# WPCLab/OpenSeg3D

Hardware: AMD Instinct MI355X
Metric: points/sec fwd+bwd, Waymo 1-sweep ~180k pts @0.1m voxel; logit parity (higher is better)
Workload: dtype f32 storage/accumulate, bf16x3 products; 1 GPU; waymo_one_sweep (BASELINE configs[1]): synthetic scene, 174633 pts/step/GPU, voxel [0.1, 0.1, 0.1], grid [1440, 1440, 64], fwd (attention dropout p=0.1, DropPath) + criterion (ohem_ce+lovasz on 3 heads) + bwd + SGD step; mode=fwdbwd, segmentor=segformer, voxels=108690, parallelism=dp1

## Files before the change

__graft_entry__.py:

```python
import os
import subprocess
import sys

ROOT = os.path.dirname(os.path.abspath(__file__))
CSRC = os.path.join(ROOT, "openseg3d_amd", "csrc")
LIB = os.path.join(CSRC, "libseg3d_hip.so")
HIP_SOURCES = ["scan.hip", "voxelize.hip", "group.hip", "rulebook.hip", "spconv.hip", "spconv_split.hip", "linear_stream.hip", "linear_x6.hip", "spconv_dma.hip", "spconv_tile.hip", "wgrad_split.hip", "wgrad_dense.hip", "wgrad_dense_lds.hip", "window.hip",
               "attention.hip", "attention_fused.hip", "attention_fused_bwd.hip", "attention_small.hip", "rownorm.hip", "segment.hip", "knn.hip", "knn_attention.hip", "class_context.hip", "loss.hip", "lovasz.hip"]
HIPCC_FLAGS = ["--offload-arch=gfx950", "-O3", "-std=c++17", "-fPIC", "-ffp-contract=off",
               "-fhip-fp32-correctly-rounded-divide-sqrt", "-Wall", "-Wno-unused-function"]


def _stale(target, deps):
    if not os.path.exists(target):
        return True
    t = os.path.getmtime(target)
    return any(os.path.getmtime(d) > t for d in deps)


def build_hip(force=False, verbose=False):
    hipcc = os.environ.get("HIPCC", "/opt/rocm/bin/hipcc")
    common = [os.path.join(CSRC, "common.hpp"), os.path.join(CSRC, "attn_common.hpp"), os.path.join(CSRC, "attn_dropout.hpp"), os.path.join(CSRC, "attn_fused.hpp"),
              os.path.join(ROOT, "include", "seg3d_hip.h")]
    objs = []
    procs = []
    for src in HIP_SOURCES:
        s = os.path.join(CSRC, src)
        o = os.path.join(CSRC, src.replace(".hip", ".o"))
        objs.append(o)
        if force or _stale(o, [s] + common):
            cmd = [hipcc] + HIPCC_FLAGS + ["-c", s, "-o", o]
            if verbose:
                print(" ".join(cmd))
            procs.append((src, subprocess.Popen(cmd, stdout=subprocess.PIPE, stderr=subprocess.STDOUT)))
    failed = False
    for src, p in procs:
        out, _ = p.communicate()
        if p.returncode != 0:
            failed = True
            sys.stderr.write(f"--- hipcc failed on {src}\n{out.decode()}\n")
        elif verbose and out.strip():
            print(out.decode())
    if failed:
        raise RuntimeError("hipcc failed")
    if force or procs or _stale(LIB, objs):
        subprocess.check_call([hipcc, "--offload-arch=gfx950", "-shared", "-fPIC", "-o", LIB] + objs)
    return LIB


def build():
    build_hip()
    subprocess.check_call(["make", "-C", os.path.join(ROOT, "oracle")], stdout=subprocess.DEVNULL)
    sys.path.insert(0, ROOT)
    import openseg3d_amd
    from openseg3d_amd import _lib
# ... 12 lines not shown
```

include/seg3d_hip.h:

```cpp
#ifndef SEG3D_HIP_H
#define SEG3D_HIP_H

#include <stddef.h>
#include <stdint.h>

#ifdef __cplusplus
extern "C" {
#endif

#define SEG3D_OK 0
#define SEG3D_EINVAL (-1)
#define SEG3D_EWORKSPACE (-2)
#define SEG3D_ELAUNCH (-3)

#define SEG3D_REDUCE_SUM 0
#define SEG3D_REDUCE_MEAN 1
#define SEG3D_REDUCE_MAX 2

int seg3d_abi_version(void);

const char* seg3d_last_error(void);

int seg3d_grid_size(const float* voxel_size, const float* range, int32_t* grid_xyz);

// ... 105 lines not shown
int seg3d_linear_pack_weight_f32(const float* weight, int32_t cin, int32_t cout, int32_t transpose,
                                 void* w_packed, void* stream);
int seg3d_linear_fwd_f32(const float* x, int64_t m, const void* w_packed, const float* bias ,
                         int32_t cin, int32_t cout, float* y, void* stream);
size_t seg3d_linear_packed_bytes_x6(int32_t cin, int32_t cout);
int seg3d_linear_pack_weight_x6(const float* weight, int32_t cin, int32_t cout, int32_t transpose, void* w_packed,
                                void* stream);
int seg3d_linear_fwd_x6(const float* x, int64_t m, const void* w_packed, const float* bias ,
                        const float* scale , const float* shift , int32_t relu, int32_t cin,
                        int32_t cout, float* y, void* stream);

typedef struct {
  const float* src;
  void* dst;
  int32_t cin, cout;
  int32_t kk, transpose, flip, reserved;
  int64_t first_block;
} seg3d_pack_job;
int seg3d_pack_weights_batched(const void* jobs, int32_t n_jobs, int64_t total_blocks, void* stream);

size_t seg3d_linear_packed_bytes(int32_t cin, int32_t cout, int32_t transpose);
int seg3d_linear_pack_weight(const float* weight, int32_t cin, int32_t cout, int32_t transpose,
                             void* w_packed, void* stream);
int seg3d_linear_fwd(const float* x, int64_t m, const void* w_packed, const float* bias ,
                     const float* addend , int32_t cin, int32_t cout,
                     float* y, void* stream);
int seg3d_linear_fwd_sum(const float* x, const float* x_add, int64_t m, const void* w_packed, const float* bias,
                         int32_t cin, int32_t cout, float* y, void* stream);
int seg3d_linear_layernorm_fwd(const float* x, int64_t m, const void* w_packed, const float* bias, const float* res,
                               const float* gamma, const float* beta, float eps, int32_t cin, int32_t cout, float* y,
                               void* stream);
int seg3d_linear_fwd_mul(const float* x, int64_t m, const void* w_packed, const float* factor, int32_t cin, int32_t cout,
                         float* y, void* stream);

size_t seg3d_window_partition_workspace_bytes(int64_t m, int32_t batch_size, const int32_t* nwin_xyz);
int seg3d_window_partition(const int32_t* coords, int64_t m, int32_t batch_size,
                           const int32_t* win_xyz, const int32_t* nwin_xyz, const int32_t* shift_xyz,
                           int32_t n_levels, const int32_t* level_lo, const int32_t* level_hi,
                           const int32_t* level_cap, int32_t* win_id, int32_t* in_win, int32_t* rank,
                           int32_t* level, int32_t* slot, int32_t* tok, int32_t* win_start,
                           int32_t* win_count, int32_t* win_tile0, int32_t* tile_item,
                           int32_t* qg_item, int32_t* counts, void* workspace,
                           size_t workspace_bytes, void* stream);

int seg3d_pos_embed(const int32_t* in_win, int64_t m, const int32_t* win_xyz ,
                    const float* inv_freq, int32_t c, float* pos, void* stream);

int seg3d_window_attn_supported(int32_t heads, int32_t dh);
size_t seg3d_window_attn_workspace_bytes(int64_t m, int32_t n_tiles, int32_t heads, int32_t dh);
int seg3d_window_attn_fwd(const float* q, const float* k, const float* v, int32_t ldq, int32_t ldk,
                          int32_t ldv, const int32_t* tok, const int32_t* win_start,
                          const int32_t* win_count, const int32_t* win_tile0,
                          const int32_t* tile_item, int32_t n_tiles, const int32_t* qg_item,
                          int32_t n_qgroups, int64_t m, int32_t n_windows, int32_t heads, int32_t dh,
                          const float* tau, float tau_min, float dropout_p, uint64_t dropout_seed, float* out,
                          float* lse, void* workspace, size_t workspace_bytes, void* stream);
int seg3d_window_attn_bwd(const float* q, const float* k, const float* v, int32_t ldq, int32_t ldk,
                          int32_t ldv, const float* out, const float* dout, const float* lse,
                          const int32_t* tok, const int32_t* win_start, const int32_t* win_count,
                          const int32_t* win_tile0, const int32_t* tile_item, int32_t n_tiles,
                          const int32_t* qg_item, int32_t n_qgroups, int64_t m, int32_t n_windows,
                          int32_t heads, int32_t dh, const float* tau,
                          float tau_min, float dropout_p, uint64_t dropout_seed, float* dq, float* dk,
                          float* dv, int32_t lddq, int32_t lddk,
                          int32_t lddv, float* dtau, void* workspace, size_t workspace_bytes,
                          void* stream);
// ... 105 lines not shown
```

openseg3d_amd/_lib.py:

```python
import ctypes
import os
import re

_HERE = os.path.dirname(os.path.abspath(__file__))
LIB_PATH = os.path.join(_HERE, "csrc", "libseg3d_hip.so")
HEADER_PATH = os.path.join(os.path.dirname(_HERE), "include", "seg3d_hip.h")

OK, EINVAL, EWORKSPACE, ELAUNCH = 0, -1, -2, -3
REDUCE_SUM, REDUCE_MEAN, REDUCE_MAX = 0, 1, 2
ABI_VERSION = 40

_p, _i32, _i64, _sz, _f = ctypes.c_void_p, ctypes.c_int32, ctypes.c_int64, ctypes.c_size_t, ctypes.c_float
_u64 = ctypes.c_uint64

SIGNATURES = {
    "seg3d_abi_version": (ctypes.c_int, []),
    "seg3d_last_error": (ctypes.c_char_p, []),
    "seg3d_grid_size": (ctypes.c_int, [_p, _p, _p]),
    "seg3d_voxelize_workspace_bytes": (_sz, [_i64]),
    "seg3d_voxelize_f32": (ctypes.c_int, [_p, _i64, _i32, _i32, _i32, _p, _p, _p, _p, _p, _p, _sz, _p]),
    "seg3d_voxelize_f64": (ctypes.c_int, [_p, _i64, _i32, _i32, _i32, _p, _p, _p, _p, _p, _p, _sz, _p]),
    "seg3d_voxelize_host_workspace_bytes": (_sz, [_i64]),
    "seg3d_voxelize_host_f32": (ctypes.c_int, [_p, _i64, _i32, _i32, _i32, _p, _p, _p, _p, _p, _p, _sz]),
    "seg3d_voxelize_host_f64": (ctypes.c_int, [_p, _i64, _i32, _i32, _i32, _p, _p, _p, _p, _p, _p, _sz]),
    "seg3d_cart2polar_f32": (ctypes.c_int, [_p, _i64, _i32, _i32, _p, _p]),
    "seg3d_cart2polar_f64": (ctypes.c_int, [_p, _i64, _i32, _i32, _p, _p]),
    "seg3d_group_index_workspace_bytes": (_sz, [_i64, _i64]),
    "seg3d_group_index": (ctypes.c_int, [_p, _i64, _i64, _p, _p, _p, _p, _sz, _p]),
    "seg3d_coord_hash_bytes": (_sz, [_i64]),
    "seg3d_coord_hash_build": (ctypes.c_int, [_p, _i64, _p, _p, _sz, _p]),
    "seg3d_rulebook_subm": (ctypes.c_int, [_p, _i64, _p, _p, _sz, _p, _p]),
    "seg3d_downsample_workspace_bytes": (_sz, [_i32, _p]),
    "seg3d_downsample_coords": (ctypes.c_int, [_p, _i64, _p, _i32, _p, _p, _i64, _p, _p, _sz, _p]),
    "seg3d_rulebook_strided": (ctypes.c_int, [_p, _i64, _i64, _p, _p, _sz, _p, _p, _p]),
    "seg3d_spconv_packed_bytes": (_sz, [_i32, _i32, _i32]),
    "seg3d_spconv_pack_weight": (ctypes.c_int, [_p, _i32, _i32, _i32, _p, _p]),
    "seg3d_spconv_fwd": (ctypes.c_int, [_p, _p, _i64, _i64, _p, _i32, _p, _i32, _i32, _p, _p, _p]),
    "seg3d_spconv_fwd_act": (ctypes.c_int, [_p, _p, _i64, _i64, _p, _i32, _p, _p, _i32, _i32, _i32, _p, _p, _p]),
    "seg3d_spconv_fwd_act_bf16": (ctypes.c_int, [_p, _i32, _p, _i64, _i64, _p, _i32, _p, _p, _i32, _i32, _i32, _p, _p, _p]),
    "seg3d_spconv_presplit_bytes": (_sz, [_i64, _i32]),
    "seg3d_spconv_presplit": (ctypes.c_int, [_p, _i64, _i32, _p, _p]),
    "seg3d_spconv_fwd_presplit": (ctypes.c_int, [_p, _p, _i64, _i64, _p, _i32, _p, _p, _i32, _i32, _i32, _p, _p, _p]),
    "seg3d_conv_plan_bytes": (_sz, [_i64]),
    "seg3d_conv_plan_workspace_bytes": (_sz, [_i64]),
    "seg3d_conv_plan_build": (ctypes.c_int, [_p, _p, _i64, _p, _p, _sz, _p]),
    "seg3d_spconv_tiled_supported": (_i32, [_i32, _i32]),
    "seg3d_spconv_fwd_tiled": (ctypes.c_int, [_p, _p, _p, _i64, _i64, _p, _i32, _p, _p, _i32, _i32, _i32, _p, _p]),
    "seg3d_spconv_fwd_tiled_bf16": (ctypes.c_int, [_p, _i32, _p, _p, _i64, _i64, _p, _i32, _p, _p, _i32, _i32, _i32, _p, _p]),
    "seg3d_debug_set_conv_nbt": (ctypes.c_int, [_i32]),
    "seg3d_debug_set_linear_stream": (ctypes.c_int, [_i32]),
    "seg3d_spconv_wgrad_workspace_bytes": (_sz, [_i64, _i32, _i32]),
    "seg3d_spconv_wgrad": (ctypes.c_int, [_p, _p, _p, _i64, _i64, _i32, _i32, _i32, _p, _p, _sz, _p]),
    "seg3d_spconv_wgrad_partials": (ctypes.c_int, [_p, _p, _p, _i64, _i64, _i32, _i32, _p, _sz, _p, _p]),
    "seg3d_spconv_wgrad_partials_xbf16": (ctypes.c_int, [_p, _p, _p, _i64, _i64, _i32, _i32, _p, _sz, _p, _p]),
    "seg3d_linear_wgrad_partials_xbf16": (ctypes.c_int, [_p, _p, _i64, _i32, _i32, _i32, _p, ctypes.c_size_t, _p, _p]),
    "seg3d_linear_packed_bytes_f32": (ctypes.c_size_t, [_i32, _i32]),
    "seg3d_linear_pack_weight_f32": (ctypes.c_int, [_p, _i32, _i32, _i32, _p, _p]),
    "seg3d_linear_fwd_f32": (ctypes.c_int, [_p, _i64, _p, _p, _i32, _i32, _p, _p]),
    "seg3d_debug_set_wgrad_lds": (ctypes.c_int, [_i32]),
    "seg3d_linear_packed_bytes_x6": (ctypes.c_size_t, [_i32, _i32]),
    "seg3d_linear_pack_weight_x6": (ctypes.c_int, [_p, _i32, _i32, _i32, _p, _p]),
    "seg3d_linear_fwd_x6": (ctypes.c_int, [_p, _i64, _p, _p, _p, _p, _i32, _i32, _i32, _p, _p]),
    "seg3d_pack_weights_batched": (ctypes.c_int, [_p, _i32, _i64, _p]),
    "seg3d_linear_wgrad_workspace_bytes": (ctypes.c_size_t, [_i64, _i32, _i32]),
    "seg3d_linear_wgrad": (ctypes.c_int, [_p, _p, _i64, _i32, _i32, _p, _p, _p, ctypes.c_size_t, _p]),
    "seg3d_linear_wgrad_partials": (ctypes.c_int, [_p, _p, _i64, _i32, _i32, _i32, _p, ctypes.c_size_t, _p, _p]),
    "seg3d_reduce_partials": (ctypes.c_int, [_p, _i32, _i64, _i64, _p, _p, _p]),
    "seg3d_reduce_partials_batched": (ctypes.c_int, [_p, _i32, _i64, _p]),
    "seg3d_linear_packed_bytes": (_sz, [_i32, _i32, _i32]),
    "seg3d_linear_pack_weight": (ctypes.c_int, [_p, _i32, _i32, _i32, _p, _p]),
    "seg3d_linear_fwd": (ctypes.c_int, [_p, _i64, _p, _p, _p, _i32, _i32, _p, _p]),
    "seg3d_linear_fwd_sum": (ctypes.c_int, [_p, _p, _i64, _p, _p, _i32, _i32, _p, _p]),
    "seg3d_linear_fwd_mul": (ctypes.c_int, [_p, _i64, _p, _p, _i32, _i32, _p, _p]),
    "seg3d_linear_layernorm_fwd": (ctypes.c_int, [_p, _i64, _p, _p, _p, _p, _p, ctypes.c_float, _i32, _i32, _p, _p]),
    "seg3d_window_partition_workspace_bytes": (_sz, [_i64, _i32, _p]),
    "seg3d_window_partition": (ctypes.c_int, [_p, _i64, _i32, _p, _p, _p, _i32, _p, _p, _p,
                                              _p, _p, _p, _p, _p, _p, _p, _p, _p, _p, _p, _p, _p, _sz, _p]),
    "seg3d_pos_embed": (ctypes.c_int, [_p, _i64, _p, _p, _i32, _p, _p]),
    "seg3d_window_attn_supported": (ctypes.c_int, [_i32, _i32]),
    "seg3d_window_attn_workspace_bytes": (_sz, [_i64, _i32, _i32, _i32]),
    "seg3d_window_attn_fwd": (ctypes.c_int, [_p, _p, _p, _i32, _i32, _i32, _p, _p, _p, _p, _p, _i32, _p, _i32,
                                             _i64, _i32, _i32, _i32, _p, _f, _f, _u64, _p, _p, _p, _sz, _p]),
    "seg3d_window_attn_bwd": (ctypes.c_int, [_p, _p, _p, _i32, _i32, _i32, _p, _p, _p, _p, _p, _p, _p, _p, _i32, _p,
                                             _i32, _i64, _i32, _i32, _i32, _p, _f, _f, _u64, _p, _p, _p, _i32, _i32, _i32,
                                             _p, _p, _sz, _p]),
    "seg3d_layernorm_fwd": (ctypes.c_int, [_p, _p, _p, _p, _p, _f, _i64, _i32, _p, _p, _p, _p]),
    "seg3d_layernorm_bwd_workspace_bytes": (ctypes.c_size_t, [_i64, _i32]),
    "seg3d_layernorm_bwd": (ctypes.c_int, [_p, _p, _p, _p, _p, _p, _i64, _i32, _p, _p, _p, _p, ctypes.c_size_t, _p]),
    "seg3d_layernorm_bwd_partials": (ctypes.c_int, [_p, _p, _p, _p, _p, _p, _i64, _i32, _p, _p, ctypes.c_size_t, _p, _p]),
    "seg3d_batchnorm_workspace_bytes": (ctypes.c_size_t, [_i64, _i32]),
    "seg3d_colstats": (ctypes.c_int, [_p, _i64, _i32, _p, _p, ctypes.c_size_t, _p]),
    "seg3d_batchnorm_stats": (ctypes.c_int, [_p, _i64, _i32, _f, _p, _p, _f, _p, _p, _p, _p, ctypes.c_size_t, _p]),
    "seg3d_affine_act": (ctypes.c_int, [_p, _p, _p, _p, _i32, _i64, _i32, _p, _p]),
    "seg3d_gelu_fwd": (ctypes.c_int, [_p, _i64, _p, _p, _p]),
    "seg3d_batchnorm_bwd": (ctypes.c_int, [_p, _p, _p, _p, _p, _p, _i32, _i64, _i32, _p, _p, _p, _p, ctypes.c_size_t, _p]),
    "seg3d_batchnorm_bwd_reduce": (ctypes.c_int, [_p, _p, _p, _p, _p, _i32, _i64, _i32, _p, _p, ctypes.c_size_t, _p]),
    "seg3d_batchnorm_bwd_apply": (ctypes.c_int, [_p, _p, _p, _p, _p, _p, _p, _p, _i32, _i64, _i32, _p, _p, _p]),
    "seg3d_segment_reduce_fwd": (ctypes.c_int, [_p, _i32, _p, _p, _i64, _i32, _p, _p, _p]),
    "seg3d_segment_reduce_bwd": (ctypes.c_int, [_p, _i32, _p, _i64, _p, _p, _i64, _i32, _p, _p]),
    "seg3d_voxel_majority_labels": (ctypes.c_int, [_p, _p, _p, _i64, _i32, _p, _p]),
    "seg3d_cross_entropy_workspace_bytes": (ctypes.c_size_t, [_i64]),
    "seg3d_cross_entropy_fwd": (ctypes.c_int, [_p, _p, _i64, _i32, _i64, _f, _p, _p, _p, ctypes.c_size_t, _p]),
    "seg3d_cross_entropy_bwd": (ctypes.c_int, [_p, _p, _p, _p, _p, _i64, _i32, _p, _p]),
    "seg3d_lovasz_workspace_bytes": (ctypes.c_size_t, [_i64, _i32]),
    "seg3d_lovasz_softmax_fwd": (ctypes.c_int, [_p, _p, _i64, _i32, _i64, _i32, _p, _p, _p, _p, _p, ctypes.c_size_t, _p]),
    "seg3d_lovasz_softmax_bwd": (ctypes.c_int, [_p, _p, _p, _p, _i64, _i32, _p, _p]),
# ... 64 lines not shown
```

openseg3d_amd/csrc/rownorm.hip:

```cpp
#include "common.hpp"

namespace {

constexpr int kThreads = 256;
constexpr int kMaxBlocks = 2048;
constexpr int kLnBwdMaxBlocks = 1024;

struct RowMap {
    int quads;
    int p;
    int items;
};

inline RowMap row_map(int c) {
    RowMap m;
    m.quads = c / 4;
    m.items = (m.quads + 63) / 64;
    int need = (m.quads + m.items - 1) / m.items;
    m.p = 8;
    while (m.p < need) m.p <<= 1;
    return m;
}

__device__ __forceinline__ float group_sum(float v, int p) {
    for (int off = 1; off < p; off <<= 1) v += __shfl_xor(v, off, SEG3D_WAVE);
    return v;
}

template <int ITEMS>
__global__ __launch_bounds__(kThreads) void ln_fwd_kernel(const float* __restrict__ x, const float* __restrict__ res,
                                                          const float* __restrict__ gamma, const float* __restrict__ beta,
                                                          const float* __restrict__ rowscale, float eps, int64_t m, int c,
                                                          RowMap rm, float* __restrict__ y, float* __restrict__ mean,
// ... 208 lines not shown
        for (; b + 96 < nblocks; b += 128) {
            s0 += part[(int64_t)b * c2 + i];
            s1 += part[(int64_t)(b + 32) * c2 + i];
            s2 += part[(int64_t)(b + 64) * c2 + i];
            s3 += part[(int64_t)(b + 96) * c2 + i];
        }
        for (; b < nblocks; b += 32) s0 += part[(int64_t)b * c2 + i];
        s = (s0 + s1) + (s2 + s3);
    }
    red[q][col] = s;
    __syncthreads();
    float t = red[0][col];
#pragma unroll
    for (int k = 1; k < 32; ++k) t += red[k][col];
    __syncthreads();
    return t;
}

__global__ __launch_bounds__(1024) void col_sums_finish(const float* __restrict__ part, int nblocks, int c,
                                                        float* __restrict__ sums ) {
    __shared__ float red[32][33];
    const int i = blockIdx.x * 32 + (threadIdx.x & 31);
    const float t = col_partial_sum(part, nblocks, 2 * c, i, red);
    if ((threadIdx.x >> 5) == 0 && i < 2 * c) sums[i] = t;
}

__global__ __launch_bounds__(kThreads) void gelu_fwd_kernel(const float* __restrict__ h, int64_t quads, float* __restrict__ g,
                                                            float* __restrict__ gp) {
    for (int64_t t = (int64_t)blockIdx.x * kThreads + threadIdx.x; t < quads; t += (int64_t)gridDim.x * kThreads) {
        const float4 v = reinterpret_cast<const float4*>(h)[t];
        const float in[4] = {v.x, v.y, v.z, v.w};
        float o[4], d[4];
#pragma unroll
        for (int i = 0; i < 4; ++i) {
            const float cdf = 0.5f * (1.0f + erff(in[i] * 0.70710678118654752440f));
            o[i] = in[i] * cdf;
            d[i] = cdf + in[i] * (0.39894228040143267794f * __expf(-0.5f * in[i] * in[i]));
        }
        reinterpret_cast<float4*>(g)[t] = make_float4(o[0], o[1], o[2], o[3]);
        if (gp) reinterpret_cast<float4*>(gp)[t] = make_float4(d[0], d[1], d[2], d[3]);
    }
}

__global__ __launch_bounds__(kThreads) void affine_act_kernel(const float* __restrict__ x, const float* __restrict__ res,
                                                              const float* __restrict__ scale, const float* __restrict__ shift,
                                                              int relu, int64_t total_quads, int quads, float* __restrict__ y) {
    for (int64_t t = (int64_t)blockIdx.x * kThreads + threadIdx.x; t < total_quads; t += (int64_t)gridDim.x * kThreads) {
        const int q = (int)(t % quads);
        const float4 xv = reinterpret_cast<const float4*>(x)[t];
        const float4 s = *reinterpret_cast<const float4*>(scale + 4 * q);
        const float4 b = *reinterpret_cast<const float4*>(shift + 4 * q);
        float4 o = make_float4(xv.x * s.x + b.x, xv.y * s.y + b.y, xv.z * s.z + b.z, xv.w * s.w + b.w);
        if (res) {
            const float4 r = reinterpret_cast<const float4*>(res)[t];
            o.x += r.x; o.y += r.y; o.z += r.z; o.w += r.w;
        }
        if (relu) {
            o.x = fmaxf(o.x, 0.f); o.y = fmaxf(o.y, 0.f); o.z = fmaxf(o.z, 0.f); o.w = fmaxf(o.w, 0.f);
        }
        reinterpret_cast<float4*>(y)[t] = o;
    }
}

__global__ __launch_bounds__(kThreads) void bn_bwd_apply_kernel(const float* __restrict__ dy, const float* __restrict__ y,
                                                                const float* __restrict__ x, const float* __restrict__ mean,
                                                                const float* __restrict__ rstd, const float* __restrict__ gamma,
                                                                const float* __restrict__ sums , int relu,
                                                                float inv_m, const float* __restrict__ inv_m_dev,
                                                                int64_t total_quads, int quads,
                                                                float* __restrict__ dx, float* __restrict__ dres) {
    const int c = quads * 4;
// ... 260 lines not shown
```

openseg3d_amd/csrc/voxelize.hip:

```cpp
#include <cstdio>

#include "common.hpp"

namespace {

constexpr int kThreads = 256;

struct VoxParams {
    int32_t grid[3];
    int32_t row_stride, xyz_col, batch_col;
};

template <typename T>
struct VoxConst {
    T lo[3];
    T vs[3];
};

__device__ __forceinline__ float floor_t(float v) { return floorf(v); }
__device__ __forceinline__ double floor_t(double v) { return floor(v); }

template <typename T>
__global__ __launch_bounds__(kThreads) void vox_insert(const T* __restrict__ pts, int64_t n, VoxParams p,
                                                       VoxConst<T> c, HashView h, uint32_t* __restrict__ slot_of) {
// ... 217 lines not shown
        const uint64_t key = (uint64_t)(((b * grid[2] + cc[2]) * grid[1] + cc[1]) * (int64_t)grid[0] + cc[0]);
        uint64_t h = key * 0x9E3779B97F4A7C15ull;
        uint64_t s = (h ^ (h >> 29)) & (cap - 1);
        while (keys[s] != key && keys[s] != ~0ull) s = (s + 1) & (cap - 1);
        if (keys[s] == ~0ull) {
            keys[s] = key;
            vals[s] = count;
            int32_t* o = voxel_coords + 4 * (int64_t)count;
            o[0] = (int32_t)b;
            o[1] = cc[2];
            o[2] = cc[1];
            o[3] = cc[0];
            ++count;
        }
        point_voxel_ids[i] = vals[s];
    }
    *n_voxels = count;
    return SEG3D_OK;
}

}

extern "C" {

int seg3d_cart2polar_f32(const float* points, int64_t n_points, int32_t row_stride, int32_t xyz_col, float* out, void* stream) {
    return cart2polar_impl<float>(points, n_points, row_stride, xyz_col, out, stream);
}

int seg3d_cart2polar_f64(const double* points, int64_t n_points, int32_t row_stride, int32_t xyz_col, double* out,
                         void* stream) {
    return cart2polar_impl<double>(points, n_points, row_stride, xyz_col, out, stream);
}

int seg3d_abi_version(void) { return 40; }

namespace {
thread_local char g_last_error[320] = "";
}

const char* seg3d_last_error(void) { return g_last_error; }

int seg3d_grid_size(const float* voxel_size, const float* range, int32_t* grid_xyz) {
    if (!voxel_size || !range || !grid_xyz) return SEG3D_EINVAL;
    for (int j = 0; j < 3; ++j) {
        volatile float span = range[3 + j] - range[j];
        volatile float g = span / voxel_size[j];
        grid_xyz[j] = (int32_t)__builtin_rintf(g);
        if (grid_xyz[j] <= 0) return SEG3D_EINVAL;
    }
    return SEG3D_OK;
}

size_t seg3d_voxelize_workspace_bytes(int64_t n_points) { return ws_bytes(n_points < 0 ? 0 : n_points); }

int seg3d_voxelize_f32(const float* points, int64_t n_points, int32_t row_stride, int32_t xyz_col, int32_t batch_col,
                       const float* voxel_size, const float* range, int32_t* voxel_coords, int32_t* point_voxel_ids,
                       int32_t* n_voxels, void* workspace, size_t workspace_bytes, void* stream) {
    return voxelize_impl<float>(points, n_points, row_stride, xyz_col, batch_col, voxel_size, range, voxel_coords,
                                point_voxel_ids, n_voxels, workspace, workspace_bytes, stream);
}

int seg3d_voxelize_f64(const double* points, int64_t n_points, int32_t row_stride, int32_t xyz_col, int32_t batch_col,
                       const float* voxel_size, const float* range, int32_t* voxel_coords, int32_t* point_voxel_ids,
                       int32_t* n_voxels, void* workspace, size_t workspace_bytes, void* stream) {
    return voxelize_impl<double>(points, n_points, row_stride, xyz_col, batch_col, voxel_size, range, voxel_coords,
                                 point_voxel_ids, n_voxels, workspace, workspace_bytes, stream);
}
// ... 27 lines not shown
```

openseg3d_amd/ops.py:

```python
import ctypes
import weakref
import os

import torch

from . import _lib
from ._lib import REDUCE_MAX, REDUCE_MEAN, REDUCE_SUM

_F3 = ctypes.c_float * 3
_F6 = ctypes.c_float * 6
_I3 = ctypes.c_int32 * 3


def _need_gpu(*tensors):
    for t in tensors:
        if t is not None and not t.is_cuda:
            raise _lib.Seg3dError("openseg3d_amd ops run on the GPU only (no CPU fallback); got a CPU tensor")


def _ptr(t):
    return None if t is None else ctypes.c_void_p(t.data_ptr())


def _stream():
# ... 1482 lines not shown
    dw = torch.empty((cout, cin), dtype=torch.float32, device=dy.device)
    db = torch.empty((cout,), dtype=torch.float32, device=dy.device) if want_db else None
    if fork is not None:
        _linear_wgrad_into(fork, x, dy, cin, cout, dw.data_ptr(), db.data_ptr() if want_db else 0)
        return dw, db
    ws_bytes = _lib.query("seg3d_linear_wgrad_workspace_bytes", x.shape[0], cin, cout)
    ws = _workspace(ws_bytes, dy.device)
    _lib.call("seg3d_linear_wgrad", _ptr(x), _ptr(dy), x.shape[0], cin, cout, _ptr(dw), _ptr(db), _ptr(ws), ws_bytes, _stream())
    return dw, db


def _linear_wgrad_into(fk, x, dy, cin, cout, dw_ptr, db_ptr, *keep):
    m = x.shape[0]
    ws_bytes = _lib.query("seg3d_linear_wgrad_workspace_bytes", m, cin, cout)
    ws = _workspace(ws_bytes, dy.device)
    chunks = ctypes.c_int32(0)
    _lib.call("seg3d_linear_wgrad_partials_xbf16" if x.dtype == torch.bfloat16 else "seg3d_linear_wgrad_partials",
              _ptr(x), _ptr(dy), m, cin, cout, 1 if db_ptr else 0, _ptr(ws), ws_bytes,
              ctypes.byref(chunks), fk.fork(ws, x, dy, *keep))
    fk.add_reduce(ws, chunks.value, cin * cout + cout, cin * cout, dw_ptr, db_ptr, *keep)


class _Ctx:

    def __init__(self, *needs):
        self.needs_input_grad = needs
        self.saved_tensors = ()

    def save_for_backward(self, *tensors):
        self.saved_tensors = tensors


GELU_SAVED_GRAD = os.environ.get("SEG3D_GELU_SAVED_GRAD", "1") != "0"


class _EncoderLayerFn(torch.autograd.Function):

    @staticmethod
    def forward(ctx, x, pos, w_in, b_in, tau, w_out, b_out, g1, be1, w1, b1, w2, b2, g2, be2, meta):
        heads, tau_min, wi, eps1, eps2, s1, s2, drop_p, drop_seed = meta
        x = _f32c(x)
        c = x.shape[1]
        live = any(ctx.needs_input_grad)
        c_in = _Ctx(live, False, live, live)
        qk, v = _AttnInProjFn.forward(c_in, x, pos, w_in, b_in)
        c_at = _Ctx(True, True, True, False, False, False)
        o = _WindowAttnPackedFn.forward(c_at, qk, v, tau, tau_min, heads, wi, drop_p, drop_seed)
        fuse_ln = (LINEAR_LN_FUSED and not live and s1 is None and s2 is None and (c // 16) in (1, 2, 3, 4, 6, 8, 12)
                   and b_out is not None and b2 is not None)
        c_n1 = _Ctx(True, True, True, True, False, False)
        if fuse_ln:
            x1 = _linear_layernorm(o, _linear_pack(w_out, 0), b_out, x, g1, be1, eps1, c, c)
        else:
            a = _linear_apply(o, _linear_pack(w_out, 0), b_out, c, c)
            x1 = _LayerNormResidualFn.forward(c_n1, a, x, g1, be1, eps1, s1)
        hid = w1.shape[0]
        h = _linear_apply(x1, _linear_pack(w1, 0), b1, c, hid)
        if live and GELU_SAVED_GRAD:
            g, gp = torch.empty_like(h), torch.empty_like(h)
            _lib.call("seg3d_gelu_fwd", _ptr(h), h.numel(), _ptr(g), _ptr(gp), _stream())
            h = gp
        else:
            g = torch.nn.functional.gelu(h)
        c_n2 = _Ctx(True, True, True, True, False, False)
        if fuse_ln:
            x2 = _linear_layernorm(g, _linear_pack(w2, 0), b2, x1, g2, be2, eps2, hid, c)
        else:
            m = _linear_apply(g, _linear_pack(w2, 0), b2, hid, c)
            x2 = _LayerNormResidualFn.forward(c_n2, m, x1, g2, be2, eps2, s2)
        ctx.parts = (c_in, c_at, c_n1, c_n2)
        ctx.save_for_backward(_saved_rows(o), _saved_rows(x1), h, _saved_rows(g), w_out, w1, w2)
        ctx.bias_params = (b_out, b1, b2)
        ctx.norm_params = (g1, be1, g2, be2)
        return x2

    @staticmethod
    def backward(ctx, dx2):
        c_in, c_at, c_n1, c_n2 = ctx.parts
        o, x1, h, g, w_out, w1, w2 = ctx.saved_tensors
        dx2 = _f32c(dx2)
        c, hid = x1.shape[1], w1.shape[0]
        fk = _WgradFork(dx2.device)
        c_n1.fork = c_n2.fork = fk
        dm, _, dg2, dbe2, _, _ = _LayerNormResidualFn.backward(c_n2, dx2)
        dw2, db2 = _linear_wgrad(g, dm, hid, c, fork=fk)
        if GELU_SAVED_GRAD:
            dh = torch.empty((dm.shape[0], hid), dtype=torch.float32, device=dm.device)
            _lib.call("seg3d_linear_fwd_mul", _ptr(dm), dm.shape[0], _ptr(_linear_pack(w2, 1)), _ptr(h), c, hid, _ptr(dh),
                      _stream())
        else:
            dh = torch.ops.aten.gelu_backward(_linear_apply(dm, _linear_pack(w2, 1), None, c, hid), h)
        dw1, db1 = _linear_wgrad(x1, dh, c, hid, fork=fk)
        d_x1 = _linear_apply(dh, _linear_pack(w1, 1), None, hid, c, addend=dx2)
        da, _, dg1, dbe1, _, _ = _LayerNormResidualFn.backward(c_n1, d_x1)
        dw_out, db_out = _linear_wgrad(o, da, c, c, fork=fk)
        do = _linear_apply(da, _linear_pack(w_out, 1), None, c, c)
        dqk, dv, dtau = _WindowAttnPackedFn.backward(c_at, do)[:3]
        c_in.dx_addend = d_x1
        dx, _, dw_in, db_in = _AttnInProjFn.backward(c_in, dqk, dv)
        b_out, b1, b2 = ctx.bias_params
        g1, be1, g2, be2 = ctx.norm_params
        fk.join((w_out, dw_out), (w1, dw1), (w2, dw2), (b_out, db_out), (b1, db1), (b2, db2), (g1, dg1), (be1, dbe1),
                (g2, dg2), (be2, dbe2))
        c_n1.fork = c_n2.fork = None
        ctx.parts = None
        return dx, None, dw_in, db_in, dtau, dw_out, db_out, dg1, dbe1, dw1, db1, dw2, db2, dg2, dbe2, None


def encoder_layer_fits(x, c, hid, heads):
    return (x.is_cuda and x.dim() == 2 and x.dtype == torch.float32 and c % 16 == 0 and hid % 16 == 0 and c <= 512
            and c % heads == 0 and CONV_PRECISION == "bf16x3")


class _SegmentReduceFn(torch.autograd.Function):
    @staticmethod
    def forward(ctx, x, seg, mode):
        x = _f32c(x)
        n, c = x.shape
        out = torch.empty((seg.n_segments, c), dtype=torch.float32, device=x.device)
        arg = torch.empty((seg.n_segments, c), dtype=torch.int32, device=x.device) if mode == REDUCE_MAX else None
        _lib.call("seg3d_segment_reduce_fwd", _ptr(x), c, _ptr(seg.order), _ptr(seg.offsets), seg.n_segments, mode,
                  _ptr(out), _ptr(arg), _stream())
        ctx.seg, ctx.mode, ctx.arg, ctx.n = seg, mode, arg, n
        return out

    @staticmethod
# ... 371 lines not shown
```

openseg3d_amd/swformer.py:

```python
import math
import os

import numpy as np

import torch
import torch.nn as nn
import torch.nn.functional as F

from . import ops


def window_geometry(sparse_shape_xyz, window_shape, do_shift):
    win = [int(w) for w in window_shape]
    if len(win) != 3:
        raise NotImplementedError("3-D windows only (config.py:68 WINDOW_SHAPE)")
    s = [float(v) for v in sparse_shape_xyz]
    nwin = [int(np.ceil(s[i] / win[i]) + 1) for i in range(3)]
    shift = [w // 2 for w in win] if do_shift else list(win)
    if s[2] == win[2]:
        shift[2] = 0
    return win, nwin, shift


class WindowPlan:
# ... 80 lines not shown
        self.tau = nn.Parameter(torch.ones(1, 1, 1))
        nn.init.xavier_uniform_(self.in_proj_weight)
        nn.init.constant_(self.out_proj.bias, 0.0)

    def drop_args(self, seed):
        if self.training and self.dropout > 0.0:
            return float(self.dropout), int(seed)
        return 0.0, 0

    def forward(self, x, pos, wi, seed=0):
        qk, v = ops.attn_in_proj(x, pos, self.in_proj_weight, self.in_proj_bias)
        drop_p, drop_seed = self.drop_args(seed)
        o = ops.window_attention_packed(qk, v, self.tau, self.tau_min, self.num_heads, wi, drop_p, drop_seed)
        return ops.linear(o, self.out_proj.weight, self.out_proj.bias)


class WindowAttention(nn.Module):
    def __init__(self, d_model, nhead, attn_drop, tau_min=0.01):
        super().__init__()
        self.self_attn = CosineMultiheadAttention(d_model, nhead, dropout=attn_drop, tau_min=tau_min)

    def forward(self, feat_2d, pos, wi, seed=0):
        return self.self_attn(feat_2d, pos, wi, seed)


class MLP(nn.Module):
    def __init__(self, in_features, hidden_features, drop=0.0):
        super().__init__()
        self.fc1 = nn.Linear(in_features, hidden_features)
        self.fc2 = nn.Linear(hidden_features, in_features)
        self.drop = drop

    def forward(self, x):
        x = F.gelu(ops.linear(x, self.fc1.weight, self.fc1.bias))
        if self.drop and self.training:
            x = F.dropout(x, self.drop)
        x = ops.linear(x, self.fc2.weight, self.fc2.bias)
        if self.drop and self.training:
            x = F.dropout(x, self.drop)
        return x


def attention_dropout_seed():
    return int(torch.randint(0, 2 ** 62, (1,), dtype=torch.int64).item())


def drop_path_scale(x, p):
    keep = 1.0 - p
    mask = x.new_empty((x.shape[0],)).bernoulli_(keep)
    if keep > 0.0:
        mask.div_(keep)
    return mask


def drop_path(x, p, training):
    if p == 0.0 or not training:
        return x
    return x * drop_path_scale(x, p).reshape((x.shape[0],) + (1,) * (x.dim() - 1))


FUSED_LAYER = os.environ.get("SEG3D_FUSED_LAYER", "1") != "0"


class EncoderLayer(nn.Module):

    def __init__(self, d_model, nhead, mlp_hidden_dim, drop=0.0, attn_drop=0.1, drop_path_rate=0.0):
# ... 59 lines not shown
```

Before: 4.195 million points/s.

## Fuse transformer FFN linear-GELU-linear into one HIP kernel for forward and backward

```diff
diff --git a/__graft_entry__.py b/__graft_entry__.py
--- a/__graft_entry__.py
+++ b/__graft_entry__.py
@@ -5,7 +5,7 @@
 ROOT = os.path.dirname(os.path.abspath(__file__))
 CSRC = os.path.join(ROOT, "openseg3d_amd", "csrc")
 LIB = os.path.join(CSRC, "libseg3d_hip.so")
-HIP_SOURCES = ["scan.hip", "voxelize.hip", "group.hip", "rulebook.hip", "spconv.hip", "spconv_split.hip", "linear_stream.hip", "linear_x6.hip", "spconv_dma.hip", "spconv_tile.hip", "wgrad_split.hip", "wgrad_dense.hip", "wgrad_dense_lds.hip", "window.hip",
+HIP_SOURCES = ["scan.hip", "voxelize.hip", "group.hip", "rulebook.hip", "spconv.hip", "spconv_split.hip", "linear_stream.hip", "linear_x6.hip", "ffn_fused.hip", "spconv_dma.hip", "spconv_tile.hip", "wgrad_split.hip", "wgrad_dense.hip", "wgrad_dense_lds.hip", "window.hip",
                "attention.hip", "attention_fused.hip", "attention_fused_bwd.hip", "attention_small.hip", "rownorm.hip", "segment.hip", "knn.hip", "knn_attention.hip", "class_context.hip", "loss.hip", "lovasz.hip"]
 HIPCC_FLAGS = ["--offload-arch=gfx950", "-O3", "-std=c++17", "-fPIC", "-ffp-contract=off",
                "-fhip-fp32-correctly-rounded-divide-sqrt", "-Wall", "-Wno-unused-function"]
@@ -20,7 +20,7 @@
 
 def build_hip(force=False, verbose=False):
     hipcc = os.environ.get("HIPCC", "/opt/rocm/bin/hipcc")
-    common = [os.path.join(CSRC, "common.hpp"), os.path.join(CSRC, "attn_common.hpp"), os.path.join(CSRC, "attn_dropout.hpp"), os.path.join(CSRC, "attn_fused.hpp"),
+    common = [os.path.join(CSRC, "common.hpp"), os.path.join(CSRC, "attn_common.hpp"), os.path.join(CSRC, "attn_dropout.hpp"), os.path.join(CSRC, "attn_fused.hpp"), os.path.join(CSRC, "gelu.hpp"),
               os.path.join(ROOT, "include", "seg3d_hip.h")]
     objs = []
     procs = []
diff --git a/include/seg3d_hip.h b/include/seg3d_hip.h
--- a/include/seg3d_hip.h
+++ b/include/seg3d_hip.h
@@ -161,6 +161,10 @@
                                void* stream);
 int seg3d_linear_fwd_mul(const float* x, int64_t m, const void* w_packed, const float* factor, int32_t cin, int32_t cout,
                          float* y, void* stream);
+int seg3d_ffn_fwd(const float* x1, int64_t m, const void* w1_packed, const float* b1, const void* w2_packed, const float* b2,
+                  int32_t c, int32_t hid, float* g, float* gp, float* y, void* stream);
+int seg3d_ffn_bwd(const float* dm, int64_t m, const float* gp, const void* w2t_packed, const void* w1t_packed, const float* dx2,
+                  int32_t c, int32_t hid, float* dh, float* dx1, void* stream);
 
 size_t seg3d_window_partition_workspace_bytes(int64_t m, int32_t batch_size, const int32_t* nwin_xyz);
 int seg3d_window_partition(const int32_t* coords, int64_t m, int32_t batch_size,
diff --git a/openseg3d_amd/_lib.py b/openseg3d_amd/_lib.py
--- a/openseg3d_amd/_lib.py
+++ b/openseg3d_amd/_lib.py
@@ -8,7 +8,7 @@
 
 OK, EINVAL, EWORKSPACE, ELAUNCH = 0, -1, -2, -3
 REDUCE_SUM, REDUCE_MEAN, REDUCE_MAX = 0, 1, 2
-ABI_VERSION = 40
+ABI_VERSION = 41
 
 _p, _i32, _i64, _sz, _f = ctypes.c_void_p, ctypes.c_int32, ctypes.c_int64, ctypes.c_size_t, ctypes.c_float
 _u64 = ctypes.c_uint64
@@ -72,6 +72,8 @@
     "seg3d_linear_fwd": (ctypes.c_int, [_p, _i64, _p, _p, _p, _i32, _i32, _p, _p]),
     "seg3d_linear_fwd_sum": (ctypes.c_int, [_p, _p, _i64, _p, _p, _i32, _i32, _p, _p]),
     "seg3d_linear_fwd_mul": (ctypes.c_int, [_p, _i64, _p, _p, _i32, _i32, _p, _p]),
+    "seg3d_ffn_fwd": (ctypes.c_int, [_p, _i64, _p, _p, _p, _p, _i32, _i32, _p, _p, _p, _p]),
+    "seg3d_ffn_bwd": (ctypes.c_int, [_p, _i64, _p, _p, _p, _p, _i32, _i32, _p, _p, _p]),
     "seg3d_linear_layernorm_fwd": (ctypes.c_int, [_p, _i64, _p, _p, _p, _p, _p, ctypes.c_float, _i32, _i32, _p, _p]),
     "seg3d_window_partition_workspace_bytes": (_sz, [_i64, _i32, _p]),
     "seg3d_window_partition": (ctypes.c_int, [_p, _i64, _i32, _p, _p, _p, _i32, _p, _p, _p,
diff --git a/openseg3d_amd/csrc/ffn_fused.hip b/openseg3d_amd/csrc/ffn_fused.hip
--- /dev/null
+++ b/openseg3d_amd/csrc/ffn_fused.hip
@@ -0,0 +1,265 @@
+#include <hip/hip_runtime.h>
+
+#include <type_traits>
+
+#include "common.hpp"
+#include "gelu.hpp"
+
+namespace {
+
+typedef float f32x4 __attribute__((ext_vector_type(4)));
+typedef float f32x2 __attribute__((ext_vector_type(2)));
+typedef __bf16 bf16x8 __attribute__((ext_vector_type(8)));
+typedef __bf16 bf16x2 __attribute__((ext_vector_type(2)));
+typedef uint32_t u32x4 __attribute__((ext_vector_type(4)));
+
+__device__ __forceinline__ uint32_t pack_bf16(float a, float b) {
+    f32x2 v = {a, b};
+    return __builtin_bit_cast(uint32_t, __builtin_convertvector(v, bf16x2));
+}
+
+__device__ __forceinline__ void split8(const f32x4& p, const f32x4& q, bf16x8* hi, bf16x8* lo) {
+    u32x4 h, l;
+    const float v[8] = {p[0], p[1], p[2], p[3], q[0], q[1], q[2], q[3]};
+#pragma unroll
+    for (int i = 0; i < 4; ++i) {
+        const uint32_t ph = pack_bf16(v[2 * i], v[2 * i + 1]);
+        const float h0 = __builtin_bit_cast(float, ph << 16);
+        const float h1 = __builtin_bit_cast(float, ph & 0xFFFF0000u);
+        h[i] = ph;
+        l[i] = pack_bf16(v[2 * i] - h0, v[2 * i + 1] - h1);
+    }
+    *hi = __builtin_bit_cast(bf16x8, h);
+    *lo = __builtin_bit_cast(bf16x8, l);
+}
+
+__device__ __forceinline__ void wave_lds_sync() {
+    __builtin_amdgcn_fence(__ATOMIC_RELEASE, "wavefront");
+    __builtin_amdgcn_wave_barrier();
+    __builtin_amdgcn_fence(__ATOMIC_ACQUIRE, "wavefront");
+}
+
+constexpr int kWaves = 8;
+constexpr int kRowsWg = kWaves * 16;
+constexpr int kHs = 36;
+
+template <int CB, int NC, int MODE>
+__global__ __launch_bounds__(512) void ffn_fused_kernel(const float* __restrict__ x, int64_t m, int c, int hid,
+                                                        const uint4* __restrict__ wa, const float* __restrict__ ba,
+                                                        const uint4* __restrict__ wb, const float* __restrict__ bb,
+                                                        const float* __restrict__ aux, const float* __restrict__ addend,
+                                                        float* __restrict__ out_a, float* __restrict__ out_b,
+                                                        float* __restrict__ y) {
+    extern __shared__ __attribute__((aligned(16))) uint4 lds[];
+    constexpr int kSlot = CB * 256 + NC * 128;
+    constexpr int kPer = (kSlot + kWaves * 64 - 1) / (kWaves * 64);
+    const int tid = threadIdx.x, lane = tid & 63, wave = tid >> 6;
+    const int g = lane >> 4, c16 = lane & 15;
+    float* hb = reinterpret_cast<float*>(lds + 2 * kSlot) + wave * (16 * kHs);
+    const int nb_a = hid >> 4, n_s = hid >> 5;
+    const int64_t row0 = (int64_t)blockIdx.x * kRowsWg + wave * 16;
+    const bool row_ok = row0 + c16 < m;
+    const int64_t arow = row_ok ? row0 + c16 : m - 1;
+    const f32x4 z = (f32x4){0.f, 0.f, 0.f, 0.f};
+
+    u32x4 wreg[kPer];
+    auto stage = [&](int t) {
+        const int s1 = t < n_s ? t : n_s - 1, s2 = t > 0 ? t - 1 : 0;
+#pragma unroll
+        for (int j = 0; j < kPer; ++j) {
+            int i = j * kWaves * 64 + tid;
+            if (kSlot % (kWaves * 64) != 0 && i >= kSlot) i = 0;
+            const uint4* src = i < CB * 256 ? wa + ((int64_t)(i >> 8) * nb_a + 2 * s1) * 128 + (i & 255)
+                                            : wb + (int64_t)s2 * NC * 128 + (i - CB * 256);
+            wreg[j] = *reinterpret_cast<const u32x4*>(src);
+        }
+    };
+    auto commit = [&](int buf) {
+#pragma unroll
+        for (int j = 0; j < kPer; ++j) {
+            const int i = j * kWaves * 64 + tid;
+            if (kSlot % (kWaves * 64) == 0 || i < kSlot) *reinterpret_cast<u32x4*>(lds + buf * kSlot + i) = wreg[j];
+        }
+    };
+
+    stage(0);
+    bf16x8 xh[CB], xl[CB];
+#pragma unroll
+    for (int cb = 0; cb < CB; ++cb) {
+        const bool in_range = cb * 32 + g * 8 < c;
+        const f32x4* p = reinterpret_cast<const f32x4*>(x + arow * c + (in_range ? cb * 32 + g * 8 : 0));
+        const f32x4 r0 = p[0], r1 = p[1];
+        split8(row_ok && in_range ? r0 : z, row_ok && in_range ? r1 : z, &xh[cb], &xl[cb]);
+    }
+    f32x4 yacc[NC];
+#pragma unroll
+    for (int n = 0; n < NC; ++n) {
+        const float b = MODE != 2 && bb ? bb[n * 16 + c16] : 0.0f;
+        yacc[n] = (f32x4){b, b, b, b};
+    }
+    commit(0);
+    __syncthreads();
+
+    bf16x8 gh = {}, gl = {};
+    int buf = 0;
+    for (int s = 0; s < n_s; ++s) {
+        const int64_t off = arow * hid + s * 32 + g * 8;
+        f32x4 hacc[2], f0, f1, d0, d1;
+        if constexpr (MODE == 2) {
+            f0 = *reinterpret_cast<const f32x4*>(aux + off);
+            f1 = *reinterpret_cast<const f32x4*>(aux + off + 4);
+            hacc[0] = hacc[1] = z;
+        } else {
+#pragma unroll
+            for (int n = 0; n < 2; ++n) {
+                const float bl = *(ba ? ba + s * 32 + n * 16 + c16 : x);
+                const float b = ba ? bl : 0.0f;
+                hacc[n] = (f32x4){b, b, b, b};
+            }
+        }
+        __builtin_amdgcn_sched_barrier(0);
+        stage(s + 1);
+        const uint4* slot = lds + buf * kSlot;
+#pragma unroll
+        for (int cb = 0; cb < CB; ++cb)
+#pragma unroll
+            for (int n = 0; n < 2; ++n) {
+                const bf16x8 bh = __builtin_bit_cast(bf16x8, slot[(cb * 2 + n) * 128 + lane]);
+                const bf16x8 bl = __builtin_bit_cast(bf16x8, slot[(cb * 2 + n) * 128 + 64 + lane]);
+                hacc[n] = __builtin_amdgcn_mfma_f32_16x16x32_bf16(xl[cb], bh, hacc[n], 0, 0, 0);
+                hacc[n] = __builtin_amdgcn_mfma_f32_16x16x32_bf16(xh[cb], bl, hacc[n], 0, 0, 0);
+                hacc[n] = __builtin_amdgcn_mfma_f32_16x16x32_bf16(xh[cb], bh, hacc[n], 0, 0, 0);
+            }
+        if (s > 0) {
+            const uint4* prev = slot + CB * 256;
+#pragma unroll
+            for (int n = 0; n < NC; ++n) {
+                const bf16x8 bh = __builtin_bit_cast(bf16x8, prev[n * 128 + lane]);
+                const bf16x8 bl = __builtin_bit_cast(bf16x8, prev[n * 128 + 64 + lane]);
+                yacc[n] = __builtin_amdgcn_mfma_f32_16x16x32_bf16(gl, bh, yacc[n], 0, 0, 0);
+                yacc[n] = __builtin_amdgcn_mfma_f32_16x16x32_bf16(gh, bl, yacc[n], 0, 0, 0);
+                yacc[n] = __builtin_amdgcn_mfma_f32_16x16x32_bf16(gh, bh, yacc[n], 0, 0, 0);
+            }
+        }
+        wave_lds_sync();
+#pragma unroll
+        for (int n = 0; n < 2; ++n)
+#pragma unroll
+            for (int r = 0; r < 4; ++r) hb[(g * 4 + r) * kHs + n * 16 + c16] = hacc[n][r];
+        wave_lds_sync();
+        f32x4 v0 = *reinterpret_cast<const f32x4*>(hb + c16 * kHs + g * 8);
+        f32x4 v1 = *reinterpret_cast<const f32x4*>(hb + c16 * kHs + g * 8 + 4);
+        if constexpr (MODE == 2) {
+            v0 = v0 * f0;
+            v1 = v1 * f1;
+        } else {
+#pragma unroll
+            for (int i = 0; i < 4; ++i) {
+                float d;
+                v0[i] = gelu_erf(v0[i], MODE == 0 ? &d : nullptr);
+                d0[i] = MODE == 0 ? d : 0.0f;
+                v1[i] = gelu_erf(v1[i], MODE == 0 ? &d : nullptr);
+                d1[i] = MODE == 0 ? d : 0.0f;
+            }
+        }
+        const f32x4 g0 = v0, g1 = v1;
+        split8(row_ok ? v0 : z, row_ok ? v1 : z, &gh, &gl);
+        commit(buf ^ 1);
+        if constexpr (MODE == 2) {
+            if (row_ok) {
+                *reinterpret_cast<f32x4*>(out_b + off) = v0;
+                *reinterpret_cast<f32x4*>(out_b + off + 4) = v1;
+            }
+        } else if constexpr (MODE == 0) {
+            if (row_ok) {
+                *reinterpret_cast<f32x4*>(out_a + off) = g0;
+                *reinterpret_cast<f32x4*>(out_a + off + 4) = g1;
+                *reinterpret_cast<f32x4*>(out_b + off) = d0;
+                *reinterpret_cast<f32x4*>(out_b + off + 4) = d1;
+            }
+        }
+        asm volatile("s_waitcnt lgkmcnt(0)\n\ts_barrier" ::: "memory");
+        buf ^= 1;
+    }
+    {
+        const uint4* prev = lds + buf * kSlot + CB * 256;
+#pragma unroll
+        for (int n = 0; n < NC; ++n) {
+            const bf16x8 bh = __builtin_bit_cast(bf16x8, prev[n * 128 + lane]);
+            const bf16x8 bl = __builtin_bit_cast(bf16x8, prev[n * 128 + 64 + lane]);
+            yacc[n] = __builtin_amdgcn_mfma_f32_16x16x32_bf16(gl, bh, yacc[n], 0, 0, 0);
+            yacc[n] = __builtin_amdgcn_mfma_f32_16x16x32_bf16(gh, bl, yacc[n], 0, 0, 0);
+            yacc[n] = __builtin_amdgcn_mfma_f32_16x16x32_bf16(gh, bh, yacc[n], 0, 0, 0);
+        }
+    }
+#pragma unroll
+    for (int r = 0; r < 4; ++r) {
+        const int64_t opos = row0 + g * 4 + r;
+        if (opos < m) {
+            float* yr = y + opos * c + c16;
+            const float* ar = MODE == 2 && addend ? addend + opos * c + c16 : nullptr;
+#pragma unroll
+            for (int n = 0; n < NC; ++n) yr[n * 16] = ar ? yacc[n][r] + ar[n * 16] : yacc[n][r];
+        }
+    }
+}
+
+template <int CB, int NC, int MODE>
+int launch_ffn(const float* x, int64_t m, int c, int hid, const void* wa, const float* ba, const void* wb, const float* bb,
+               const float* aux, const float* addend, float* out_a, float* out_b, float* y, hipStream_t st) {
+    constexpr size_t kSlotBytes = (size_t)(CB * 256 + NC * 128) * 16;
+    constexpr size_t lds = 2 * kSlotBytes + (size_t)kWaves * 16 * kHs * 4;
+    static_assert(lds <= 160 * 1024, "LDS per CU");
+    auto kernel = ffn_fused_kernel<CB, NC, MODE>;
+    static bool raised = false;
+    if (!raised && lds > 64 * 1024) {
+        SEG3D_CHECK_HIP(hipFuncSetAttribute(reinterpret_cast<const void*>(kernel), hipFuncAttributeMaxDynamicSharedMemorySize,
+                                            (int)lds));
+        raised = true;
+    }
+    hipLaunchKernelGGL(kernel, dim3((unsigned)ceil_div64(m, kRowsWg)), dim3(kWaves * 64), lds, st, x, m, c, hid,
+                       reinterpret_cast<const uint4*>(wa), ba, reinterpret_cast<const uint4*>(wb), bb, aux, addend, out_a,
+                       out_b, y);
+    SEG3D_CHECK_LAUNCH();
+    return SEG3D_OK;
+}
+
+template <int MODE>
+int dispatch_ffn(const float* x, int64_t m, int c, int hid, const void* wa, const float* ba, const void* wb, const float* bb,
+                 const float* aux, const float* addend, float* out_a, float* out_b, float* y, hipStream_t st) {
+    switch (c) {
+        case 48: return launch_ffn<2, 3, MODE>(x, m, c, hid, wa, ba, wb, bb, aux, addend, out_a, out_b, y, st);
+        case 96: return launch_ffn<3, 6, MODE>(x, m, c, hid, wa, ba, wb, bb, aux, addend, out_a, out_b, y, st);
+        case 192: return launch_ffn<6, 12, MODE>(x, m, c, hid, wa, ba, wb, bb, aux, addend, out_a, out_b, y, st);
+        default: return SEG3D_EINVAL;
+    }
+}
+
+bool ffn_shape_ok(int64_t m, int32_t c, int32_t hid) {
+    return m >= 0 && (c == 48 || c == 96 || c == 192) && hid > 0 && hid % 32 == 0;
+}
+
+}
+
+extern "C" {
+
+int seg3d_ffn_fwd(const float* x1, int64_t m, const void* w1_packed, const float* b1, const void* w2_packed, const float* b2,
+                  int32_t c, int32_t hid, float* g, float* gp, float* y, void* stream) {
+    if (!ffn_shape_ok(m, c, hid) || !w1_packed || !w2_packed || (!g) != (!gp)) return SEG3D_EINVAL;
+    if (m == 0) return SEG3D_OK;
+    if (!x1 || !y) return SEG3D_EINVAL;
+    if (g)
+        return dispatch_ffn<0>(x1, m, c, hid, w1_packed, b1, w2_packed, b2, nullptr, nullptr, g, gp, y, as_stream(stream));
+    return dispatch_ffn<1>(x1, m, c, hid, w1_packed, b1, w2_packed, b2, nullptr, nullptr, nullptr, nullptr, y,
+                           as_stream(stream));
+}
+
+int seg3d_ffn_bwd(const float* dm, int64_t m, const float* gp, const void* w2t_packed, const void* w1t_packed, const float* dx2,
+                  int32_t c, int32_t hid, float* dh, float* dx1, void* stream) {
+    if (!ffn_shape_ok(m, c, hid) || !w2t_packed || !w1t_packed) return SEG3D_EINVAL;
+    if (m == 0) return SEG3D_OK;
+    if (!dm || !gp || !dh || !dx1) return SEG3D_EINVAL;
+    return dispatch_ffn<2>(dm, m, c, hid, w2t_packed, nullptr, w1t_packed, nullptr, gp, dx2, nullptr, dh, dx1, as_stream(stream));
+}
+
+}
diff --git a/openseg3d_amd/csrc/gelu.hpp b/openseg3d_amd/csrc/gelu.hpp
--- /dev/null
+++ b/openseg3d_amd/csrc/gelu.hpp
@@ -0,0 +1,8 @@
+#pragma once
+#include <hip/hip_runtime.h>
+
+__device__ __forceinline__ float gelu_erf(float h, float* gp) {
+    const float cdf = 0.5f * (1.0f + erff(h * 0.70710678118654752440f));
+    if (gp) *gp = cdf + h * (0.39894228040143267794f * __expf(-0.5f * h * h));
+    return h * cdf;
+}
diff --git a/openseg3d_amd/csrc/rownorm.hip b/openseg3d_amd/csrc/rownorm.hip
--- a/openseg3d_amd/csrc/rownorm.hip
+++ b/openseg3d_amd/csrc/rownorm.hip
@@ -1,4 +1,5 @@
 #include "common.hpp"
+#include "gelu.hpp"
 
 namespace {
 
@@ -273,11 +274,7 @@
         const float in[4] = {v.x, v.y, v.z, v.w};
         float o[4], d[4];
 #pragma unroll
-        for (int i = 0; i < 4; ++i) {
-            const float cdf = 0.5f * (1.0f + erff(in[i] * 0.70710678118654752440f));
-            o[i] = in[i] * cdf;
-            d[i] = cdf + in[i] * (0.39894228040143267794f * __expf(-0.5f * in[i] * in[i]));
-        }
+        for (int i = 0; i < 4; ++i) o[i] = gelu_erf(in[i], &d[i]);
         reinterpret_cast<float4*>(g)[t] = make_float4(o[0], o[1], o[2], o[3]);
         if (gp) reinterpret_cast<float4*>(gp)[t] = make_float4(d[0], d[1], d[2], d[3]);
     }
diff --git a/openseg3d_amd/csrc/voxelize.hip b/openseg3d_amd/csrc/voxelize.hip
--- a/openseg3d_amd/csrc/voxelize.hip
+++ b/openseg3d_amd/csrc/voxelize.hip
@@ -273,7 +273,7 @@
     return cart2polar_impl<double>(points, n_points, row_stride, xyz_col, out, stream);
 }
 
-int seg3d_abi_version(void) { return 40; }
+int seg3d_abi_version(void) { return 41; }
 
 namespace {
 thread_local char g_last_error[320] = "";
diff --git a/openseg3d_amd/ops.py b/openseg3d_amd/ops.py
--- a/openseg3d_amd/ops.py
+++ b/openseg3d_amd/ops.py
@@ -1538,6 +1538,20 @@
 
 
 GELU_SAVED_GRAD = os.environ.get("SEG3D_GELU_SAVED_GRAD", "1") != "0"
+FFN_FUSED = os.environ.get("SEG3D_FFN_FUSED", "1") != "0"
+
+
+def ffn_fits(c, hid, backward=False):
+    return (FFN_FUSED and c in ((48, 96) if backward else (48, 96, 192)) and hid % 32 == 0
+            and CONV_PRECISION == "bf16x3")
+
+
+def ffn_apply(x, w1, b1, w2, b2, g=None, gp=None):
+    c, hid = w1.shape[1], w1.shape[0]
+    y = torch.empty((x.shape[0], c), dtype=torch.float32, device=x.device)
+    _lib.call("seg3d_ffn_fwd", _ptr(x), x.shape[0], _ptr(_linear_pack(w1, 0)), _ptr(b1), _ptr(_linear_pack(w2, 0)), _ptr(b2),
+              c, hid, _ptr(g), _ptr(gp), _ptr(y), _stream())
+    return y
 
 
 class _EncoderLayerFn(torch.autograd.Function):
@@ -1561,18 +1575,25 @@
             a = _linear_apply(o, _linear_pack(w_out, 0), b_out, c, c)
             x1 = _LayerNormResidualFn.forward(c_n1, a, x, g1, be1, eps1, s1)
         hid = w1.shape[0]
-        h = _linear_apply(x1, _linear_pack(w1, 0), b1, c, hid)
-        if live and GELU_SAVED_GRAD:
-            g, gp = torch.empty_like(h), torch.empty_like(h)
-            _lib.call("seg3d_gelu_fwd", _ptr(h), h.numel(), _ptr(g), _ptr(gp), _stream())
-            h = gp
+        fused_ffn = live and GELU_SAVED_GRAD and ffn_fits(c, hid)
+        if fused_ffn:
+            g = torch.empty((x1.shape[0], hid), dtype=torch.float32, device=x1.device)
+            h = torch.empty_like(g)
+            m = ffn_apply(x1, w1, b1, w2, b2, g, h)
         else:
-            g = torch.nn.functional.gelu(h)
+            h = _linear_apply(x1, _linear_pack(w1, 0), b1, c, hid)
+            if live and GELU_SAVED_GRAD:
+                g, gp = torch.empty_like(h), torch.empty_like(h)
+                _lib.call("seg3d_gelu_fwd", _ptr(h), h.numel(), _ptr(g), _ptr(gp), _stream())
+                h = gp
+            else:
+                g = torch.nn.functional.gelu(h)
         c_n2 = _Ctx(True, True, True, True, False, False)
         if fuse_ln:
             x2 = _linear_layernorm(g, _linear_pack(w2, 0), b2, x1, g2, be2, eps2, hid, c)
         else:
-            m = _linear_apply(g, _linear_pack(w2, 0), b2, hid, c)
+            if not fused_ffn:
+                m = _linear_apply(g, _linear_pack(w2, 0), b2, hid, c)
             x2 = _LayerNormResidualFn.forward(c_n2, m, x1, g2, be2, eps2, s2)
         ctx.parts = (c_in, c_at, c_n1, c_n2)
         ctx.save_for_backward(_saved_rows(o), _saved_rows(x1), h, _saved_rows(g), w_out, w1, w2)
@@ -1590,14 +1611,22 @@
         c_n1.fork = c_n2.fork = fk
         dm, _, dg2, dbe2, _, _ = _LayerNormResidualFn.backward(c_n2, dx2)
         dw2, db2 = _linear_wgrad(g, dm, hid, c, fork=fk)
-        if GELU_SAVED_GRAD:
+        d_x1 = None
+        if GELU_SAVED_GRAD and ffn_fits(c, hid, backward=True):
+            dh = torch.empty((dm.shape[0], hid), dtype=torch.float32, device=dm.device)
+            d_x1 = torch.empty((dm.shape[0], c), dtype=torch.float32, device=dm.device)
+            _lib.call("seg3d_ffn_bwd", _ptr(dm), dm.shape[0], _ptr(h), _ptr(_linear_pack(w2, 1)), _ptr(_linear_pack(w1, 1)),
+                      _ptr(dx2), c, hid, _ptr(dh), _ptr(d_x1), _stream())
+            dw1, db1 = _linear_wgrad(x1, dh, c, hid, fork=fk)
+        elif GELU_SAVED_GRAD:
             dh = torch.empty((dm.shape[0], hid), dtype=torch.float32, device=dm.device)
             _lib.call("seg3d_linear_fwd_mul", _ptr(dm), dm.shape[0], _ptr(_linear_pack(w2, 1)), _ptr(h), c, hid, _ptr(dh),
                       _stream())
         else:
             dh = torch.ops.aten.gelu_backward(_linear_apply(dm, _linear_pack(w2, 1), None, c, hid), h)
-        dw1, db1 = _linear_wgrad(x1, dh, c, hid, fork=fk)
-        d_x1 = _linear_apply(dh, _linear_pack(w1, 1), None, hid, c, addend=dx2)
+        if d_x1 is None:
+            dw1, db1 = _linear_wgrad(x1, dh, c, hid, fork=fk)
+            d_x1 = _linear_apply(dh, _linear_pack(w1, 1), None, hid, c, addend=dx2)
         da, _, dg1, dbe1, _, _ = _LayerNormResidualFn.backward(c_n1, d_x1)
         dw_out, db_out = _linear_wgrad(o, da, c, c, fork=fk)
         do = _linear_apply(da, _linear_pack(w_out, 1), None, c, c)
diff --git a/openseg3d_amd/swformer.py b/openseg3d_amd/swformer.py
--- a/openseg3d_amd/swformer.py
+++ b/openseg3d_amd/swformer.py
@@ -136,6 +136,9 @@
         self.drop = drop
 
     def forward(self, x):
+        if (not torch.is_grad_enabled() and not self.drop and x.is_cuda and x.dim() == 2 and x.dtype == torch.float32
+                and ops.ffn_fits(x.shape[1], self.fc1.out_features)):
+            return ops.ffn_apply(x.contiguous(), self.fc1.weight, self.fc1.bias, self.fc2.weight, self.fc2.bias)
         x = F.gelu(ops.linear(x, self.fc1.weight, self.fc1.bias))
         if self.drop and self.training:
             x = F.dropout(x, self.drop)
```

Measured after the change: 4.252 million points/s, median of 6. +1.4%, better.
